# ha7ilm/csdr

Measured on AMD Instinct MI355X. Metric: complex MS/s in->out, WFM demod chain @2.4 MS/s x N streams, higher is better.
Workload: dtype f32

## Files before the change

csdr_amd/__init__.py:

```python
import ctypes as C
import os
import sys
import subprocess
import numpy as np

HERE = os.path.dirname(os.path.abspath(__file__))
LIB_PATH = os.environ.get("CSDR_AMD_LIB") or os.path.join(HERE, "libcsdr_amd.so")
ROOT = os.path.dirname(HERE)

c64 = np.complex64
f32 = np.float32

SHIFT = {"addition": 0, "math": 1, "table": 2, "unroll": 3, "addfast": 4}
WINDOWS = {"BOXCAR": 0, "BLACKMAN": 1, "HAMMING": 2}


class CsdrAmdError(RuntimeError):
    pass


def build(verbose=False):
    r = subprocess.run(["make", "-C", os.path.join(HERE, "csrc"), "-j8"], capture_output=True, text=True)
    if r.returncode != 0:
        raise CsdrAmdError("libcsdr_amd build failed:\n" + r.stdout[-4000:] + r.stderr[-4000:])
# ... 305 lines not shown
    L.csdr_amd_loopback_destroy.argtypes = [vp]; L.csdr_amd_loopback_destroy.restype = None
    L.csdr_amd_loopback_abort.argtypes = [vp]; L.csdr_amd_loopback_abort.restype = None
    L.csdr_amd_comm_create_loopback.restype = vp; L.csdr_amd_comm_create_loopback.argtypes = [vp, vp, i]
    L.csdr_amd_comm_create_null.restype = vp; L.csdr_amd_comm_create_null.argtypes = [vp, i, i]
    L.csdr_amd_comm_create_ipc.restype = vp; L.csdr_amd_comm_create_ipc.argtypes = [vp, C.c_char_p, i, i]
    L.csdr_amd_fastddc_inv_kernel_name.restype = C.c_char_p; L.csdr_amd_fastddc_inv_kernel_name.argtypes = [vp]
    L.csdr_amd_fastddc_inv_kernels.restype = C.c_char_p; L.csdr_amd_fastddc_inv_kernels.argtypes = [vp]
    L.csdr_amd_fastddc_inv_set_profiling.argtypes = [vp, i]
    L.csdr_amd_fastddc_inv_kernel_time.argtypes = [vp, C.POINTER(C.c_double), C.POINTER(C.c_long)]
    L.csdr_amd_fastddc_inv_stage_time.argtypes = [vp, i, C.POINTER(C.c_double), C.POINTER(C.c_long)]
    L.csdr_amd_wfm_create.restype = vp; L.csdr_amd_wfm_create.argtypes = [vp, i, fl, i, vp, i, i, fl, i, sz]
    L.csdr_amd_wfm_destroy.argtypes = [vp]
    L.csdr_amd_wfm_reset.argtypes = [vp]
    L.csdr_amd_wfm_process.restype = C.c_long; L.csdr_amd_wfm_process.argtypes = [vp, vp, sz, sz, vp, vp, sz]
    L.csdr_amd_wfm_kernel_name.restype = C.c_char_p; L.csdr_amd_wfm_kernel_name.argtypes = [vp]
    ll = C.c_longlong; db = C.c_double
    L.csdr_amd_wfm_ring_create.restype = vp; L.csdr_amd_wfm_ring_create.argtypes = [vp, i, fl, i, vp, i, i, fl, i, sz, i]
    L.csdr_amd_wfm_ring_destroy.argtypes = [vp]; L.csdr_amd_wfm_ring_destroy.restype = None
    L.csdr_amd_wfm_ring_reset.argtypes = [vp]
    L.csdr_amd_wfm_ring_acquire.argtypes = [vp, ll, db]
    L.csdr_amd_wfm_ring_input.restype = vp; L.csdr_amd_wfm_ring_input.argtypes = [vp, ll, C.POINTER(sz)]
    L.csdr_amd_wfm_ring_submit.restype = ll; L.csdr_amd_wfm_ring_submit.argtypes = [vp]
    L.csdr_amd_wfm_ring_wait.restype = C.c_long; L.csdr_amd_wfm_ring_wait.argtypes = [vp, ll, db]
    L.csdr_amd_wfm_ring_output.restype = vp; L.csdr_amd_wfm_ring_output.argtypes = [vp, ll, C.POINTER(sz)]
    L.csdr_amd_wfm_ring_set_rate.argtypes = [vp, fl]
    L.csdr_amd_wfm_ring_get_rate.restype = fl; L.csdr_amd_wfm_ring_get_rate.argtypes = [vp]
    L.csdr_amd_wfm_ring_set_timeouts.argtypes = [vp, db, db]
    L.csdr_amd_wfm_ring_resident.argtypes = [vp]
    L.csdr_amd_wfm_ring_stop.argtypes = [vp]
    L.csdr_amd_wfm_ring_slots.argtypes = [vp]
# ... 2610 lines not shown
```

csdr_amd/csrc/wfm.hip:

```cpp
#include "common.hpp"
#include "wfm_mfma.hpp"
#include "seeds.hpp"
#include <math.h>
#include <stdlib.h>
#include <vector>
#include <string>
#include <string.h>
using namespace csdr_amd;

namespace {

constexpr int HIST = WFM_HIST;
constexpr int TILE_A = 64;
constexpr int WARM = 48;

struct WfmParams {
    int D, L, F;
    int T;
    long long B;
    long long j_first;
    int n_audio;
};

__device__ __forceinline__ float u8_to_f(uint32_t v) { return fmaf((float)v, 0x1.010102p-7f, -1.0f); }
// ... 149 lines not shown
    bool ended;
    std::string kernel_name;
    bool profiling;
    KernelTimer timer;
    double prof_ms; long prof_launches;
    bool use_mfma;
    WfmMfmaDevice mfma;
    DevBuf<> seq_frags; DevBuf<float> seq_cum; DevBuf<float2> dtab;
    DevBuf<float2> d_ctab; size_t ctab_cap;
    float2 c_prev;
    long long tab_first; bool tab_valid;
    long tabs_built;
    bool ps; std::vector<float> rates, h_taps; DevBuf<float> d_scales;
    DevBuf<float2> d_dtab_old; DevBuf<int> d_lead_n; int *d_list; DevBuf<float> d_lead_d; std::vector<int> retuned;
    Owned<csdr_amd::SeedTables, seeds_destroy> seeds;
};

extern "C" {

static int wfm_upload_stream_tables(csdr_amd_wfm *w, int s, float rate)
{
    WfmMfmaTable t;
    wfm_mfma_build_table(w->D, w->L, w->F, rate, w->h_taps.data(), t);
    CSDR_HIP(hipMemcpy((uint8_t *)w->mfma.d_seq_frags + (size_t)s * t.seq_frags.size(), t.seq_frags.data(), t.seq_frags.size(), hipMemcpyHostToDevice));
    CSDR_HIP(hipMemcpy(w->mfma.d_seq_cum + (size_t)s * t.seq_cum.size(), t.seq_cum.data(), t.seq_cum.size() * sizeof(float), hipMemcpyHostToDevice));
    CSDR_HIP(hipMemcpy(w->mfma.d_dtab + (size_t)s * t.dtab.size(), t.dtab.data(), t.dtab.size() * sizeof(float2), hipMemcpyHostToDevice));
    CSDR_HIP(hipMemcpy(w->d_scales.get() + s, &t.seq_scale, sizeof(float), hipMemcpyHostToDevice));
    return 0;
}

// ... 115 lines not shown
    CSDR_HIP(hipMemsetAsync(w->d_last[1].get(), 0, sizeof(float) * w->n_streams, st));
    if (w->d_rot) CSDR_HIP(hipMemsetAsync(w->d_rot.get(), 0, sizeof(cf32) * (HIST + w->max_block + 64), st));
    if (w->d_hist) CSDR_HIP(hipMemsetAsync(w->d_hist.get(), 0x80, (size_t)2 * HIST * w->n_streams, st));
    for (int k = 0; k < 2; k++) if (w->d_head[k]) CSDR_HIP(hipMemsetAsync(w->d_head[k].get(), 0x80, wfm_mfma_head_bytes(w->n_streams), st));
    w->hflip = 0;
    w->B = 0; w->next_j = 0; w->last_T = 0; w->flip = 0; w->ended = false;
    w->c_prev = make_float2(1.f, 0.f); w->tab_valid = false; w->tab_first = 0;
    w->retuned.clear();
    if (w->seeds) { const int rc = seeds_reset(w->seeds.get()); if (rc) return rc; }
    return 0;
}

const char *csdr_amd_wfm_kernel_name(const csdr_amd_wfm *w) { return w->kernel_name.c_str(); }
int csdr_amd_wfm_fallback(const csdr_amd_wfm *w) { return w->use_mfma ? 0 : 1; }

int csdr_amd_wfm_seed_stats(const csdr_amd_wfm *w, long out[5])
{
    if (!w || !out) return fail_msg(-3, "wfm_seed_stats: bad arguments");
    if (!w->ps) return fail_msg(-3, "wfm_seed_stats: the object shares one rate, it has no per-stream seed tables (csdr_amd_wfm_tables_built counts its host-built table)");
    seeds_stats(w->seeds.get(), out);
    return 0;
}

long csdr_amd_wfm_tables_built(const csdr_amd_wfm *w)
{
    if (!w) return fail_msg(-3, "wfm_tables_built: bad arguments");
    if (!w->ps) return w->tabs_built;
    long st[5]; seeds_stats(w->seeds.get(), st);
    return st[0];
}
// ... 94 lines not shown
                if (n_lead > n_audio) n_lead = n_audio;
            }
            if (n_lead > 0) {
                const int nr = (int)w->retuned.size(), S = w->n_streams;
                if (!w->d_lead_n) { CSDR_HIP(dev_alloc(w->d_lead_n, sizeof(int) * 2 * S)); w->d_list = w->d_lead_n.get() + S; CSDR_HIP(dev_alloc(w->d_lead_d, sizeof(float) * (size_t)lead_max * S)); }
                int *hl = (int *)c->pinned_acquire(sizeof(int) * (size_t)(S + nr)); if (!hl) return -2;
                for (int s = 0; s < S; s++) hl[s] = 0;
                for (int k = 0; k < nr; k++) { hl[w->retuned[k]] = (int)n_lead; hl[S + k] = w->retuned[k]; }
                rc = c->pinned_upload(w->d_lead_n.get(), sizeof(int) * (size_t)(S + nr)); if (rc) return rc;
                rc = wfm_mfma_lead(st, in, in_pitch, back.head_in, w->d_taps.get(), sv.ctab, sv.pitch, w->mfma.d_dtab, w->d_dtab_old.get(), w->d_list, nr, w->d_lead_d.get(), lead_max,
                                   w->D, w->L, w->F, w->B, w->next_j, (int)n_lead);
                if (rc) return rc;
                psa.d_lead_d = w->d_lead_d.get(); psa.d_lead_n = w->d_lead_n.get();
            }
        }
        rc = wfm_mfma_launch(st, e0, e1, in, in_pitch, w->mfma, ctab_call, w->n_streams, T, w->B, w->next_j, n_audio, back, w->ps ? &psa : nullptr);
        if (rc) return rc;
        if (n_audio > 0) w->retuned.clear();
        w->hflip ^= 1;
        if (n_audio > 0) w->flip ^= 1;
    } else {
        if ((size_t)n_audio + 40 > w->demod_pitch) return fail_msg(-3, "wfm: internal audio buffer too small");
        if (n_audio > 0) {
            WfmParams p; p.D = w->D; p.L = w->L; p.F = w->F; p.T = T; p.B = w->B; p.j_first = w->next_j; p.n_audio = n_audio;
            const int span = w->D * (w->F * (TILE_A - 1) + 1) + w->L + 16;
            const size_t lds = (size_t)((span + 7) / 8 * 8 + 2 * TILE_A) * sizeof(float2) + 64;
            if (lds > 64 * 1024) { const int arc = lds_attr_once((const void *)k_wfm_front, lds); if (arc) return arc; }
            if (e0) CSDR_HIP(hipEventRecord(e0, st));
            hipLaunchKernelGGL(k_wfm_front, dim3(w->n_streams, cdiv(n_audio, TILE_A)), dim3(256), lds, st,
                               in, in_pitch, w->d_hist.get(), w->d_rot.get(), w->d_taps.get(), w->d_demod.get(), w->demod_pitch, p);
            CSDR_LAUNCH_CHECK();
// ... 18 lines not shown
```

csdr_amd/csrc/wfm_mfma.hip:

```cpp
#include "common.hpp"
#include "wfm_mfma.hpp"
#include <hip/hip_ext.h>
#include <math.h>
#include <string.h>
#include <stdlib.h>
#include <complex>
#include <vector>
using namespace csdr_amd;

namespace csdr_amd {

bool wfm_mfma_supported(int D, int L, int F)
{
    if ((D * F) & 1) return false;
    const int win_off = (18 * D) & ~15;
    const int span_bytes = 2 * (D * (3 * F + 10) + L) - win_off;
    if (span_bytes > 64 * WFM_NK) return false;
    if (D + L + 3 * D * F + 8 > WFM_HIST) return false;
    return true;
}

void wfm_mfma_build_table(int D, int L, int F, float shift_rate, const float *taps, WfmMfmaTable &t)
{
    t.D = D; t.L = L; t.F = F;
// ... 97 lines not shown
            for (int l = 0; l < 3; l++) acc[l] = __builtin_amdgcn_mfma_i32_16x16x64_i8(A[ks * 3 + l], Bf[ks], acc[l], 0, 0, 0);
        }
    }
}

struct SeqParams {
    int n_streams; long long B2; long long tile_first; int n_tiles, tiles_per_seg;
    int stride, win_off; float scale;
    long long two_T;
    float alpha; const float *last_in; float *last_out; int16_t *s16; float *af; size_t out_pitch; long long j_first; int n_audio;
    const uint8_t *head_in; uint8_t *head_out;
    long long col_bytes; int col_chunks, col_audio, n_cols;
    size_t frag_stride, tab_pitch; int tab_len;
    const float *scales;
    const float *lead_d; const int *lead_n; int lead_stride;
};

#ifndef SEQ_RB_KIB
#define SEQ_RB_KIB 9
#endif
constexpr int SEQ_RB = 1024 * SEQ_RB_KIB;
#ifndef SEQ_RING_PAD
#define SEQ_RING_PAD 32
#endif
constexpr int SEQ_RP = SEQ_RB + SEQ_RING_PAD;
constexpr int SEQ_NGR = 4 * WFM_NK;
#ifndef SEQ_TPG_N
#define SEQ_TPG_N 6
#endif
#ifndef SEQ_NLD_N
// ... 29 lines not shown
    unsigned *cnt;
    unsigned long long *t_first;
    unsigned long long *next_item;
    unsigned *exiting;
    const uint8_t *in_ring; int16_t *out_ring; size_t in_slot_bytes, out_slot_elems;
    int n_slots, desc_lines, n_wsb, T, D, L, F;
    long long idle_ticks, life_ticks;
    const float *lead_d; int lead_stride;
    const float *lead_state;
    unsigned long long *stats;
    int fence_mode;
};
__device__ __forceinline__ uint32_t sys_load(const uint32_t *p) { return __hip_atomic_load(p, __ATOMIC_RELAXED, __HIP_MEMORY_SCOPE_SYSTEM); }
__device__ __forceinline__ uint32_t res_tag(long long k) { return (uint32_t)((unsigned long long)k % 0xfffffffeull) + 1u; }

template <bool PS, bool RES = false>
__global__ __launch_bounds__(64 * SEQ_NW) void k_wfm_mfma_seq(const uint8_t *__restrict__ in, size_t in_pitch, const v4i *__restrict__ frags, const float *__restrict__ cum,
                                                               const float2 *__restrict__ dtab, const float2 *__restrict__ ctab, SeqParams p_in, ResCtl rc)
{
    static_assert(!(PS && RES), "the resident form exists for the shared-rate kernel");
    constexpr int TPG = SEQ_TPG, SPW = 16 / SEQ_NLW, NTHR = 64 * SEQ_NW;
    extern __shared__ float4 lds_raw[];
    uint8_t *lds_in = reinterpret_cast<uint8_t *>(lds_raw);
    float *lds_out = reinterpret_cast<float *>(lds_in + 16 * SEQ_RP);
    float *lcum = lds_out + 16 * SEQ_OUTP;
    float2 *ctl = reinterpret_cast<float2 *>(lcum + (SEQ_NGR + 1) * 16);
    const int tid = threadIdx.x, wv = __builtin_amdgcn_readfirstlane(tid >> 6), lane = tid & 63, col = lane & 15, q = lane >> 4;
    const bool fetches = wv >= TPG;
#ifdef WFM_PROF
    const long long t_entry = __builtin_readcyclecounter();
    long long t_first = t_entry, t_last = t_entry;
#endif
    const int fw = wv - TPG;
    float scale = p_in.scale;
    if constexpr (PS) { const int sbp = blockIdx.x; frags += (size_t)sbp * p_in.frag_stride; cum += (size_t)sbp * ((SEQ_NGR + 1) * 16); dtab += (size_t)sbp * 3072; ctab += sbp; scale = p_in.scales[sbp]; }
    for (int i = tid; i < (SEQ_NGR + 1) * 16; i += NTHR) lcum[i] = cum[i];
    v4i A[WFM_NK * 3];
#pragma unroll
    for (int s = 0; s < WFM_NK * 3; s++) A[s] = frags[s * 64 + lane];

    float c_lo[4], c_hi[4];
    {
        const float4 a = *reinterpret_cast<const float4 *>(cum + 4 * q), b = *reinterpret_cast<const float4 *>(cum + (size_t)SEQ_NGR * 16 + 4 * q);
        c_lo[0] = a.x; c_lo[1] = a.y; c_lo[2] = a.z; c_lo[3] = a.w; c_hi[0] = b.x; c_hi[1] = b.y; c_hi[2] = b.z; c_hi[3] = b.w;
    }
    const float K = 0.340447550238101026565118445432744920253753662109375f;
    SeqParams p_res;
    if constexpr (RES) p_res = p_in;
    const SeqParams &p = RES ? p_res : p_in;
    unsigned long long item = 0;
    long long res_t_launch = 0;
    uint32_t *const rctl = reinterpret_cast<uint32_t *>(ctl);
    const float2 *const lseed = ctl + 1;
    long long st_wait = 0, st_body = 0, st_done = 0, st_items = 0, st_t = 0;
    if constexpr (RES) { item = rc.next_item[blockIdx.x]; res_t_launch = wall_clock64(); st_t = res_t_launch; }
    bool pend = false; unsigned pend_c = 0; int pend_slot = 0, pend_n = 0; long long pend_k = 0;
    uint32_t pre_v[4] = {0u, 0u, 0u, 0u}; bool pre_valid = false;
    auto res_complete = [&]() {
        if constexpr (RES) {
            if (tid == 0 && pend) {
                pend = false;
                if (pend_c + 1 == (unsigned)rc.n_wsb) {
                    const unsigned long long tf = __hip_atomic_exchange(rc.t_first + pend_slot, ~0ull, __ATOMIC_RELAXED, __HIP_MEMORY_SCOPE_AGENT), td = (unsigned long long)wall_clock64();
                    __hip_atomic_store(rc.cnt + pend_slot, 0u, __ATOMIC_RELAXED, __HIP_MEMORY_SCOPE_AGENT);
                    uint32_t *dn = rc.done + (size_t)pend_slot * 16;
                    __hip_atomic_store(dn + 1, (uint32_t)pend_n, __ATOMIC_RELAXED, __HIP_MEMORY_SCOPE_SYSTEM);
                    __hip_atomic_store(dn + 2, (uint32_t)tf, __ATOMIC_RELAXED, __HIP_MEMORY_SCOPE_SYSTEM); __hip_atomic_store(dn + 3, (uint32_t)(tf >> 32), __ATOMIC_RELAXED, __HIP_MEMORY_SCOPE_SYSTEM);
                    __hip_atomic_store(dn + 4, (uint32_t)td, __ATOMIC_RELAXED, __HIP_MEMORY_SCOPE_SYSTEM); __hip_atomic_store(dn + 5, (uint32_t)(td >> 32), __ATOMIC_RELAXED, __HIP_MEMORY_SCOPE_SYSTEM);
                    asm volatile("s_waitcnt vmcnt(0)" ::: "memory");
                    __hip_atomic_store(dn, res_tag(pend_k), __ATOMIC_RELAXED, __HIP_MEMORY_SCOPE_SYSTEM);
// ... 66 lines not shown
        auto j_hi = [&](long long kk) -> long long {
            if (kk < 0) return -1;
            const long long avail_last = (kk + 1) * rc.T - 1;
            if (avail_last - (rc.L - 1) < 0) return -1;
            const long long k_max = (avail_last - (rc.L - 1)) / rc.D;
            return k_max >= 10 ? (k_max - 10) / rc.F : -1;
        };
        const long long jp = j_hi(res_k - 1), jn = j_hi(res_k);
        p_res.B2 = 2 * res_k * rc.T;
        p_res.j_first = jp + 1; p_res.n_audio = (int)(jn - jp);
        p_res.tile_first = p_res.j_first / 4; p_res.n_tiles = (int)((p_res.j_first + p_res.n_audio - 1) / 4 - p_res.tile_first + 1);
        p_res.tiles_per_seg = p_res.n_tiles;
        p_res.s16 = rc.out_ring + (size_t)res_slot * rc.out_slot_elems;
        if (tid == 0) (void)__hip_atomic_fetch_min(rc.t_first + res_slot, (unsigned long long)wall_clock64(), __ATOMIC_RELAXED, __HIP_MEMORY_SCOPE_AGENT);
    }
    const int sb = RES ? (int)(item % (unsigned)rc.n_wsb) : (int)blockIdx.x;
    const int seg_y = RES ? 0 : (int)blockIdx.y;
    const int col0 = PS ? 16 * seg_y : 0;
    if constexpr (RES) {
        in = rc.in_ring + (size_t)res_slot * rc.in_slot_bytes;
        pblock = rc.in_ring + (size_t)((res_slot + rc.n_slots - 1) % rc.n_slots) * rc.in_slot_bytes + (long long)sb * 16 * (long long)in_pitch;
    }
    const long long t0 = p.tile_first + (long long)seg_y * p.tiles_per_seg * (PS ? 16 : 1);
    long long t1 = t0 + p.tiles_per_seg; if (t1 > p.tile_first + p.n_tiles) t1 = p.tile_first + p.n_tiles;
    if (!RES && t0 >= t1) return;
    const int n_it = (int)(t1 - t0), n_grp = (n_it + TPG - 1) / TPG;
    const int n_lead = RES ? res_lead : ((PS && p.lead_n && seg_y == 0) ? p.lead_n[sb] : 0);
    const int n_warm = RES ? ((res_k > 0 && !res_retuned) ? 2 : 0) : ((PS || seg_y > 0) ? 2 : 0);
    const int last_stream = p.n_streams - 1;
    const int tstride = p.stride;
    const long long org = PS ? (long long)col0 * p.col_bytes : 0LL;
    long long wg = (t0 - (long long)n_warm * TPG) * tstride + p.win_off - p.B2 - org;
// ... 177 lines not shown
            const int srow = ei / SPS, k = ei % SPS, kr = g * SPS + k;
            if (ei >= 16 * SPS) continue;
            if (PS ? (kr < col_lo(srow) || kr >= col_hi(srow)) : (kr < seg_lo || kr >= seg_hi || s0 + srow >= p.n_streams)) continue;
            const float e = lds_out[srow * SEQ_OUTP + (g % SEQ_OUTS) * SPS + k];
            const long long idx = idx0 + kr;
            const size_t at = PS ? (size_t)sb * p.out_pitch + (size_t)srow * p.col_audio + idx : (size_t)(s0 + srow) * p.out_pitch + idx;
            p.s16[at] = (int16_t)s16_of(e);
            if (p.af) p.af[at] = e;
        }
    };
#ifdef WFM_PROF
    long long prof[8] = {0, 0, 0, 0, 0, 0, 0, 0}, t_prev = __builtin_readcyclecounter();
#endif
    if (fetches) {
        typedef unsigned wfm_u4 __attribute__((ext_vector_type(4)));
        constexpr int NST = RES ? 8 : 44;
#define WFM_ST_ALL(X) X(0) X(1) X(2) X(3) X(4) X(5) X(6) X(7) X(8) X(9) X(10) X(11) X(12) X(13) X(14) X(15) X(16) X(17) X(18) X(19) X(20) X(21) X(22) X(23) \
                      X(24) X(25) X(26) X(27) X(28) X(29) X(30) X(31) X(32) X(33) X(34) X(35) X(36) X(37) X(38) X(39) X(40) X(41) X(42) X(43)
#define X(k) wfm_u4 st##k = {0u, 0u, 0u, 0u};
        WFM_ST_ALL(X)
#undef X
        int n_st = 0, st_n0 = 0;
        const int srow = 8 * fw + (lane >> 3), pc = lane & 7;
        const int lo_r = col_lo(srow), hi_r = col_hi(srow);
        const bool row_ok = PS ? hi_r > lo_r : s0 + srow < p.n_streams;
        const size_t row_at = PS ? (size_t)sb * p.out_pitch + (size_t)srow * p.col_audio : (size_t)(s0 + srow) * p.out_pitch;
        int16_t *const orow = p.s16 + row_at;
        auto flush = [&]() __attribute__((always_inline)) {
            if constexpr (PS) {
#define X(j) if (j < NST && j < n_st && row_ok) { const int a = st_n0 + SEQ_LINE * j + 8 * pc;                                                             \
                 if (a + 8 <= hi_r) *reinterpret_cast<uint4 *>(orow + (idx0 + a)) = make_uint4(st##j[0], st##j[1], st##j[2], st##j[3]);        \
// ... 56 lines not shown
            if (gi + 1 < n_grp) { while (F < F_end && F + 1024 <= wg_n + SEQ_RB) row_step(); }
            PROF_T(3)
            if (WFM_DIAG < 4) take_line(gi - 1);
            PROF_T(4)
#ifdef WFM_PROF
            prof[6] += 1;
#endif
            wg = wg_n;
        }
#ifdef WFM_PROF
        if (lane == 0) for (int k = 0; k < 8; k++) atomicAdd(&g_wfm_prof[wv][k], (unsigned long long)prof[k]);
        t_last = __builtin_readcyclecounter();
#endif
        __syncthreads();
        if (WFM_DIAG < 4) { take_line(n_grp - 1); take_line(n_grp); flush(); }
#undef WFM_ST_ALL
    } else {
    PROF_T(7)
#ifdef WFM_PROF
    t_first = __builtin_readcyclecounter();
#endif
    for (int gi = -n_warm; gi < n_grp; gi++) {
        const int it = gi * TPG + wv;
        float *lout = lds_out + ((gi + SEQ_OUTS) % SEQ_OUTS) * SPS;
        if (it < n_it && (WFM_DIAG < 3)) {
            const long long ws = wg + (long long)wv * tstride;
            const long long n0 = (ws + p.B2) >> 1;
            const int off = (int)(n0 & 1023);
            const bool two = off + 32 * WFM_NK > 1024;
            const int bo = 2 * (1024 - off);
// ... 117 lines not shown
    }
#ifdef WFM_PROF
    if (lane == 0) for (int k = 0; k < 8; k++) atomicAdd(&g_wfm_prof[wv][k], (unsigned long long)prof[k]);
    t_last = __builtin_readcyclecounter();
#endif
    __syncthreads();
    if (!emit_vec) emit_scalar(n_grp - 1);
    }
    if (PS && seg_y + 1 == (int)gridDim.y) {
        if (iir_lane && col0 + lane == p.n_cols - 1) p.last_out[sb] = yst;
        if (tid < 32 && p.two_T >= 512 && (p.two_T & 15) == 0) {
            const uint4 v = *reinterpret_cast<const uint4 *>(in + (size_t)sb * in_pitch + (p.two_T - 512) + 16 * tid);
            *reinterpret_cast<uint4 *>(p.head_out + (size_t)sb * SEQ_HEAD + 512 + 16 * tid) = v;
        }
    } else
    if (!PS && !RES && seg_y + 1 == (int)gridDim.y) {
        if (iir_lane && s0 + lane < p.n_streams) p.last_out[s0 + lane] = yst;
        if (tid < 16 * 32 && p.two_T >= 512 && (p.two_T & 15) == 0 && s0 + tid / 32 < p.n_streams) {
            const int srow = tid / 32, piece = tid % 32;
            const uint4 v = *reinterpret_cast<const uint4 *>(sblock + (size_t)srow * in_pitch + (p.two_T - 512) + 16 * piece);
            *reinterpret_cast<uint4 *>(p.head_out + (size_t)(s0 + srow) * SEQ_HEAD + 512 + 16 * piece) = v;
        }
    }
#ifdef WFM_PROF
    if (lane == 0) {
        asm volatile("s_waitcnt vmcnt(0)" ::: "memory");
        const long long t_exit = __builtin_readcyclecounter();
        atomicAdd(&g_wfm_life[wv][0], (unsigned long long)(t_first - t_entry)); atomicAdd(&g_wfm_life[wv][1], (unsigned long long)(t_last - t_first));
        atomicAdd(&g_wfm_life[wv][2], (unsigned long long)(t_exit - t_last)); atomicAdd(&g_wfm_life[wv][3], 1ULL);
    }
#endif
    if constexpr (!RES) break;
    else {
        if (tid == 0) { const long long t = wall_clock64(); st_body += t - st_t; st_t = t; }
        if (wv == 0) {
            const unsigned long long nx = item + gridDim.x;
            const long long nk = (long long)(nx / (unsigned)rc.n_wsb);
            const uint32_t *dsc = rc.desc + (size_t)(nk % rc.n_slots) * rc.desc_lines * 16;
            const int nd = rc.desc_lines * 16;
#pragma unroll
            for (int j = 0; j < 4; j++) { const int d = lane + 64 * j; pre_v[j] = d < nd ? sys_load(dsc + d) : 0u; }
            pre_valid = true;
        }
        if (rc.fence_mode == 2) __threadfence_system();
        if (wv != 0 || !emit_vec) asm volatile("s_waitcnt vmcnt(0)" ::: "memory");
        __syncthreads();
        if (tid == 0) {
// ... 81 lines not shown
                         const float2 *d_dtab_old, const int *d_list, int n_list, float *d_lead_d, int lead_stride, float *d_warm, float *d_state, float alpha,
                         int D, int L, int F, long long B, long long j_first, int n_lead)
{
    if (n_list <= 0) return 0;
    if (j_first < RES_WARM) return fail_msg(-3, "wfm ring: a retune needs %d audio samples in front of the block", RES_WARM);
    LeadParams lp; lp.D = D; lp.L = L; lp.F = F; lp.B = B; lp.j_first = j_first; lp.n_lead = n_lead; lp.tab_pitch = 1; lp.dtab_stride = 0;
    lp.ct_stride = 0; lp.head_pitch = in_pitch; lp.head_off = two_T - 512; lp.c_first = (B >> 10) - 4; lp.ja0 = -RES_WARM; lp.warm = d_warm; lp.lead_stride = lead_stride;
    hipLaunchKernelGGL(k_wfm_lead, dim3(n_lead + RES_WARM, n_list), dim3(128), 0, st, in, in_pitch, prev, d_taps, ctab, d_dtab, d_dtab_old, d_list, d_lead_d, lp);
    CSDR_LAUNCH_CHECK();
    hipLaunchKernelGGL(k_wfm_lead_state, dim3((n_list + 63) / 64), dim3(64), 0, st, d_warm, d_state, n_list, alpha);
    CSDR_LAUNCH_CHECK();
    return 0;
}

int wfm_mfma_launch(hipStream_t st, hipEvent_t ev_begin, hipEvent_t ev_end, const uint8_t *in, size_t in_pitch, const WfmMfmaDevice &dev, const float2 *ctab,
                    int n_streams, int T, long long B, long long j_first, int n_audio, const WfmBackArgs &back, const WfmPerStream *ps)
{
    if (in_pitch * 16 + 4096 >= ((size_t)1 << 32)) return fail_msg(-3, "wfm: in_pitch %zu too large for the matrix-core front end (32-bit row offsets)", in_pitch);
    if (n_audio <= 0) {
        hipLaunchKernelGGL(k_wfm_roll_head, dim3(n_streams), dim3(256), 0, st, in, in_pitch, 2LL * T, back.head_in, back.head_out);
        CSDR_LAUNCH_CHECK();
        return 0;
    }
    SeqParams sp;
    memset((void *)&sp, 0, sizeof sp);
    ResCtl no_res; memset((void *)&no_res, 0, sizeof no_res);
    sp.n_streams = n_streams; sp.B2 = 2 * B; sp.two_T = 2LL * T;
    sp.tile_first = j_first / 4; sp.n_tiles = (int)((j_first + n_audio - 1) / 4 - sp.tile_first + 1);
    sp.stride = dev.tile_stride_bytes; sp.win_off = dev.win_off_bytes; sp.scale = dev.seq_scale;
    const int n_cu = current_device_cu_count();
    const int n_wsb = (n_streams + 15) / 16;
    int n_seg = (n_cu + n_wsb - 1) / n_wsb; if (n_seg < 1) n_seg = 1;
// ... 13 lines not shown
        int np = (n_per + 16 * n_ss - 1) / (16 * n_ss); if (np < 1) np = 1;
        sp.tiles_per_seg = np * tpp;
        sp.n_cols = (sp.n_tiles + sp.tiles_per_seg - 1) / sp.tiles_per_seg;
        n_seg = (sp.n_cols + 15) / 16;
        sp.col_bytes = (long long)sp.tiles_per_seg * sp.stride; sp.col_chunks = (int)(sp.col_bytes / 2048); sp.col_audio = 4 * sp.tiles_per_seg;
        sp.frag_stride = (size_t)WFM_NK * 3 * 64; sp.tab_pitch = ps->tab_pitch; sp.tab_len = ps->tab_len; sp.scales = ps->d_scales;
        sp.lead_d = ps->d_lead_d; sp.lead_n = ps->d_lead_n; sp.lead_stride = ps->lead_stride;
        if (sp.col_bytes * 16 + 4096 >= (1LL << 32)) return fail_msg(-3, "wfm: block too large for the per-stream kernel's 32-bit row offsets");
        const size_t ldsp = (size_t)16 * SEQ_RP + 16 * SEQ_OUTP * sizeof(float) + (SEQ_NGR + 1) * 16 * sizeof(float) + 2 * 48 * sizeof(float2);
        { const int arc = lds_attr_once((const void *)k_wfm_mfma_seq<true>, ldsp); if (arc) return arc; }
        if (ev_begin && ev_end)
            hipExtLaunchKernelGGL(k_wfm_mfma_seq<true>, dim3(n_streams, n_seg), dim3(64 * SEQ_NW), ldsp, st, ev_begin, ev_end, 0, in, in_pitch, (const v4i *)dev.d_seq_frags, dev.d_seq_cum, dev.d_dtab, ctab, sp, no_res);
        else
            hipLaunchKernelGGL(k_wfm_mfma_seq<true>, dim3(n_streams, n_seg), dim3(64 * SEQ_NW), ldsp, st, in, in_pitch, (const v4i *)dev.d_seq_frags, dev.d_seq_cum, dev.d_dtab, ctab, sp, no_res);
        CSDR_LAUNCH_CHECK();
        if (T < 256 || (T & 7)) {
            hipLaunchKernelGGL(k_wfm_roll_head, dim3(n_streams), dim3(256), 0, st, in, in_pitch, 2LL * T, back.head_in, back.head_out);
            CSDR_LAUNCH_CHECK();
        }
        return 0;
    }
    const size_t lds = (size_t)16 * SEQ_RP + 16 * SEQ_OUTP * sizeof(float) + (SEQ_NGR + 1) * 16 * sizeof(float);
    { const int arc = lds_attr_once((const void *)k_wfm_mfma_seq<false>, lds); if (arc) return arc; }
    if (ev_begin && ev_end)
        hipExtLaunchKernelGGL(k_wfm_mfma_seq<false>, dim3(n_wsb, n_seg), dim3(64 * SEQ_NW), lds, st, ev_begin, ev_end, 0, in, in_pitch, (const v4i *)dev.d_seq_frags, dev.d_seq_cum, dev.d_dtab, ctab, sp, no_res);
    else
        hipLaunchKernelGGL(k_wfm_mfma_seq<false>, dim3(n_wsb, n_seg), dim3(64 * SEQ_NW), lds, st, in, in_pitch, (const v4i *)dev.d_seq_frags, dev.d_seq_cum, dev.d_dtab, ctab, sp, no_res);
    CSDR_LAUNCH_CHECK();
    if (T < 256 || (T & 7)) {
        hipLaunchKernelGGL(k_wfm_roll_head, dim3(n_streams), dim3(256), 0, st, in, in_pitch, 2LL * T, back.head_in, back.head_out);
        CSDR_LAUNCH_CHECK();
    }
    return 0;
}

int wfm_mfma_launch_resident(hipStream_t st, hipEvent_t ev_end, const WfmMfmaDevice &dev, int n_streams, size_t in_pitch, float alpha, size_t out_pitch, const WfmResident &rv, int grid)
{
// ... 83 lines not shown
```

csdr_amd/csrc/wfm_mfma.hpp:

```cpp
#pragma once
#include "common.hpp"
#include <vector>

namespace csdr_amd {

constexpr int WFM_HIST = 256;
constexpr int WFM_NK = 8;

struct WfmMfmaTable {
    int D, L, F, tile_stride_bytes, win_off_bytes;
    std::vector<int8_t> seq_frags;
    std::vector<float> seq_cum;
    std::vector<float2> dtab;
    float seq_scale;
};

struct WfmMfmaDevice {
    int tile_stride_bytes, win_off_bytes;
    void *d_seq_frags; float *d_seq_cum; float2 *d_dtab; float seq_scale;
};

struct WfmBackArgs {
    float alpha; const float *last_in; float *last_out; int16_t *s16; float *af; size_t out_pitch; const uint8_t *head_in; uint8_t *head_out;
};
// ... 8 lines not shown
    int n_slots, desc_lines, T, D, L, F;
    long long idle_ticks, life_ticks;
    const float *lead_d, *lead_state; int lead_stride;
    unsigned long long *stats; int fence_mode;
};
constexpr int WFM_RES_WARM = 48;
int wfm_mfma_launch_resident(hipStream_t st, hipEvent_t ev_end, const WfmMfmaDevice &dev, int n_streams, size_t in_pitch, float alpha, size_t out_pitch, const WfmResident &rv, int grid);
int wfm_resident_max_grid();
int wfm_mfma_lead_shared(hipStream_t st, const uint8_t *in, size_t in_pitch, const uint8_t *prev, size_t two_T, const float *d_taps, const float2 *ctab, const float2 *d_dtab,
                         const float2 *d_dtab_old, const int *d_list, int n_list, float *d_lead_d, int lead_stride, float *d_warm, float *d_state, float alpha,
                         int D, int L, int F, long long B, long long j_first, int n_lead);

bool wfm_mfma_supported(int D, int L, int F);
void wfm_mfma_build_table(int D, int L, int F, float shift_rate, const float *taps, WfmMfmaTable &t);
size_t wfm_mfma_head_bytes(int n_streams);
int wfm_mfma_launch(hipStream_t st, hipEvent_t ev_begin, hipEvent_t ev_end, const uint8_t *in, size_t in_pitch, const WfmMfmaDevice &dev, const float2 *ctab,
                    int n_streams, int T, long long B, long long j_first, int n_audio, const WfmBackArgs &back, const WfmPerStream *ps = nullptr);
int wfm_mfma_lead(hipStream_t st, const uint8_t *in, size_t in_pitch, const uint8_t *head, const float *d_taps, const float2 *ctab, size_t tab_pitch, const float2 *d_dtab,
                  const float2 *d_dtab_old, const int *d_list, int n_list, float *d_lead_d, int lead_stride, int D, int L, int F, long long B, long long j_first, int n_lead);

}
```

include/csdr_amd.h:

```cpp
#ifndef CSDR_AMD_H
#define CSDR_AMD_H
#include <stddef.h>
#include <stdint.h>

#ifdef __cplusplus
extern "C" {
#endif

typedef struct csdr_complexf_s { float i, q; } csdr_complexf;

typedef enum { CSDR_WINDOW_BOXCAR = 0, CSDR_WINDOW_BLACKMAN = 1, CSDR_WINDOW_HAMMING = 2 } csdr_window_t;

typedef struct csdr_amd_ctx csdr_amd_ctx;

csdr_amd_ctx *csdr_amd_ctx_create(int device, void *hip_stream);
void          csdr_amd_ctx_destroy(csdr_amd_ctx *ctx);
int           csdr_amd_ctx_sync(csdr_amd_ctx *ctx);
void         *csdr_amd_ctx_stream(csdr_amd_ctx *ctx);
const char   *csdr_amd_last_error(void);
int           csdr_amd_device_count(void);
const char   *csdr_amd_device_arch(csdr_amd_ctx *ctx);

void *csdr_amd_malloc(csdr_amd_ctx *ctx, size_t bytes);
void  csdr_amd_free(csdr_amd_ctx *ctx, void *dptr);
// ... 568 lines not shown
typedef struct csdr_amd_wfm csdr_amd_wfm;
csdr_amd_wfm *csdr_amd_wfm_create(csdr_amd_ctx *ctx, int n_streams, float shift_rate, int decimation,
                                  const float *host_taps, int taps_length, int frac_rate,
                                  float tau, int audio_rate, size_t max_block_samples);
csdr_amd_wfm *csdr_amd_wfm_create_rates(csdr_amd_ctx *ctx, int n_streams, const float *shift_rates, int decimation,
                                        const float *host_taps, int taps_length, int frac_rate,
                                        float tau, int audio_rate, size_t max_block_samples);
int   csdr_amd_wfm_set_rate(csdr_amd_wfm *w, int stream, float shift_rate);
float csdr_amd_wfm_get_rate(const csdr_amd_wfm *w, int stream);
void csdr_amd_wfm_destroy(csdr_amd_wfm *w);
int  csdr_amd_wfm_reset(csdr_amd_wfm *w);
long csdr_amd_wfm_process(csdr_amd_wfm *w, const uint8_t *in, size_t in_pitch, size_t block_samples,
                          int16_t *audio_s16, float *audio_f, size_t out_pitch);
const char *csdr_amd_wfm_kernel_name(const csdr_amd_wfm *w);
int csdr_amd_wfm_fallback(const csdr_amd_wfm *w);
int  csdr_amd_wfm_seed_stats(const csdr_amd_wfm *w, long out[5]);
long csdr_amd_wfm_tables_built(const csdr_amd_wfm *w);
int csdr_amd_wfm_set_profiling(csdr_amd_wfm *w, int on);
int csdr_amd_wfm_kernel_time(csdr_amd_wfm *w, double *total_ms, long *launches);

typedef struct csdr_amd_wfm_ring csdr_amd_wfm_ring;
csdr_amd_wfm_ring *csdr_amd_wfm_ring_create(csdr_amd_ctx *ctx, int n_streams, float shift_rate, int decimation, const float *host_taps, int taps_length, int frac_rate,
                                            float tau, int audio_rate, size_t block_samples, int n_slots);
void csdr_amd_wfm_ring_destroy(csdr_amd_wfm_ring *r);
int  csdr_amd_wfm_ring_reset(csdr_amd_wfm_ring *r);
int  csdr_amd_wfm_ring_acquire(csdr_amd_wfm_ring *r, long long seq, double timeout_s);
uint8_t *csdr_amd_wfm_ring_input(csdr_amd_wfm_ring *r, long long seq, size_t *pitch_bytes);
long long csdr_amd_wfm_ring_submit(csdr_amd_wfm_ring *r);
long csdr_amd_wfm_ring_wait(csdr_amd_wfm_ring *r, long long seq, double timeout_s);
const int16_t *csdr_amd_wfm_ring_output(csdr_amd_wfm_ring *r, long long seq, size_t *pitch_samples);
// ... 114 lines not shown
```

Baseline: 2.933 million.

## Add persistent grid-stride walk launch for shared-rate WFM matrix-core kernel

Adds a WALK variant of the sequential MFMA WFM kernel. It launches one workgroup per CU by default and has each workgroup loop over (stream-block, segment) items with a grid stride. Fetch waves skip loading the A fragments and cum tables, and the fetch-side staging register count drops from 44 to 36, which frees registers and overlaps setup. The last-segment tail work (IIR state, head copy) is moved into the walk loop. This is meant to cut launch and tail overhead when there are more items than CUs, at the cost of serializing items per workgroup and extra barriers.

Result: no change. 2.926 million (-0.2%).

```diff
diff --git a/csdr_amd/__init__.py b/csdr_amd/__init__.py
--- a/csdr_amd/__init__.py
+++ b/csdr_amd/__init__.py
@@ -343,6 +343,9 @@
     L.csdr_amd_wfm_reset.argtypes = [vp]
     L.csdr_amd_wfm_process.restype = C.c_long; L.csdr_amd_wfm_process.argtypes = [vp, vp, sz, sz, vp, vp, sz]
     L.csdr_amd_wfm_kernel_name.restype = C.c_char_p; L.csdr_amd_wfm_kernel_name.argtypes = [vp]
+    if hasattr(L, "csdr_amd_wfm_set_walk"):
+        L.csdr_amd_wfm_set_walk.argtypes = [vp, i]
+        L.csdr_amd_wfm_last_launch.argtypes = [vp, C.POINTER(C.c_int), C.POINTER(C.c_int)]
     ll = C.c_longlong; db = C.c_double
     L.csdr_amd_wfm_ring_create.restype = vp; L.csdr_amd_wfm_ring_create.argtypes = [vp, i, fl, i, vp, i, i, fl, i, sz, i]
     L.csdr_amd_wfm_ring_destroy.argtypes = [vp]; L.csdr_amd_wfm_ring_destroy.restype = None
diff --git a/csdr_amd/csrc/wfm.hip b/csdr_amd/csrc/wfm.hip
--- a/csdr_amd/csrc/wfm.hip
+++ b/csdr_amd/csrc/wfm.hip
@@ -187,6 +187,8 @@
     bool ps; std::vector<float> rates, h_taps; DevBuf<float> d_scales;
     DevBuf<float2> d_dtab_old; DevBuf<int> d_lead_n; int *d_list; DevBuf<float> d_lead_d; std::vector<int> retuned;
     Owned<csdr_amd::SeedTables, seeds_destroy> seeds;
+    int walk = 0;
+    WfmLaunchInfo last_launch = {0, 0};
 };
 
 extern "C" {
@@ -332,6 +334,21 @@
 const char *csdr_amd_wfm_kernel_name(const csdr_amd_wfm *w) { return w->kernel_name.c_str(); }
 int csdr_amd_wfm_fallback(const csdr_amd_wfm *w) { return w->use_mfma ? 0 : 1; }
 
+int csdr_amd_wfm_set_walk(csdr_amd_wfm *w, int grid)
+{
+    if (!w || grid < -1) return fail_msg(-3, "wfm_set_walk: bad arguments");
+    w->walk = grid;
+    return 0;
+}
+
+int csdr_amd_wfm_last_launch(const csdr_amd_wfm *w, int *workgroups, int *items)
+{
+    if (!w) return fail_msg(-3, "wfm_last_launch: bad arguments");
+    if (workgroups) *workgroups = w->last_launch.workgroups;
+    if (items) *items = w->last_launch.items;
+    return 0;
+}
+
 int csdr_amd_wfm_seed_stats(const csdr_amd_wfm *w, long out[5])
 {
     if (!w || !out) return fail_msg(-3, "wfm_seed_stats: bad arguments");
@@ -456,7 +473,8 @@
                 psa.d_lead_d = w->d_lead_d.get(); psa.d_lead_n = w->d_lead_n.get();
             }
         }
-        rc = wfm_mfma_launch(st, e0, e1, in, in_pitch, w->mfma, ctab_call, w->n_streams, T, w->B, w->next_j, n_audio, back, w->ps ? &psa : nullptr);
+        rc = wfm_mfma_launch(st, e0, e1, in, in_pitch, w->mfma, ctab_call, w->n_streams, T, w->B, w->next_j, n_audio, back, w->ps ? &psa : nullptr,
+                             w->walk, &w->last_launch);
         if (rc) return rc;
         if (n_audio > 0) w->retuned.clear();
         w->hflip ^= 1;
diff --git a/csdr_amd/csrc/wfm_mfma.hip b/csdr_amd/csrc/wfm_mfma.hip
--- a/csdr_amd/csrc/wfm_mfma.hip
+++ b/csdr_amd/csrc/wfm_mfma.hip
@@ -135,6 +135,7 @@
     size_t frag_stride, tab_pitch; int tab_len;
     const float *scales;
     const float *lead_d; const int *lead_n; int lead_stride;
+    int walk_wsb, walk_items;
 };
 
 #ifndef SEQ_RB_KIB
@@ -194,11 +195,12 @@
 __device__ __forceinline__ uint32_t sys_load(const uint32_t *p) { return __hip_atomic_load(p, __ATOMIC_RELAXED, __HIP_MEMORY_SCOPE_SYSTEM); }
 __device__ __forceinline__ uint32_t res_tag(long long k) { return (uint32_t)((unsigned long long)k % 0xfffffffeull) + 1u; }
 
-template <bool PS, bool RES = false>
+template <bool PS, bool RES = false, bool WALK = false>
 __global__ __launch_bounds__(64 * SEQ_NW) void k_wfm_mfma_seq(const uint8_t *__restrict__ in, size_t in_pitch, const v4i *__restrict__ frags, const float *__restrict__ cum,
                                                                const float2 *__restrict__ dtab, const float2 *__restrict__ ctab, SeqParams p_in, ResCtl rc)
 {
     static_assert(!(PS && RES), "the resident form exists for the shared-rate kernel");
+    static_assert(!WALK || (!PS && !RES), "the walk belongs to the launched shared-rate kernel");
     constexpr int TPG = SEQ_TPG, SPW = 16 / SEQ_NLW, NTHR = 64 * SEQ_NW;
     extern __shared__ float4 lds_raw[];
     uint8_t *lds_in = reinterpret_cast<uint8_t *>(lds_raw);
@@ -208,21 +210,24 @@
     const int tid = threadIdx.x, wv = __builtin_amdgcn_readfirstlane(tid >> 6), lane = tid & 63, col = lane & 15, q = lane >> 4;
     const bool fetches = wv >= TPG;
 #ifdef WFM_PROF
-    const long long t_entry = __builtin_readcyclecounter();
+    long long t_entry = __builtin_readcyclecounter();
     long long t_first = t_entry, t_last = t_entry;
 #endif
     const int fw = wv - TPG;
     float scale = p_in.scale;
     if constexpr (PS) { const int sbp = blockIdx.x; frags += (size_t)sbp * p_in.frag_stride; cum += (size_t)sbp * ((SEQ_NGR + 1) * 16); dtab += (size_t)sbp * 3072; ctab += sbp; scale = p_in.scales[sbp]; }
-    for (int i = tid; i < (SEQ_NGR + 1) * 16; i += NTHR) lcum[i] = cum[i];
+    constexpr bool FETCH_FIRST = WALK;
     v4i A[WFM_NK * 3];
-#pragma unroll
-    for (int s = 0; s < WFM_NK * 3; s++) A[s] = frags[s * 64 + lane];
-
-    float c_lo[4], c_hi[4];
-    {
+    float c_lo[4] = {0.f, 0.f, 0.f, 0.f}, c_hi[4] = {0.f, 0.f, 0.f, 0.f};
+    if (!FETCH_FIRST || !fetches) {
+        for (int i = tid; i < (SEQ_NGR + 1) * 16; i += (FETCH_FIRST ? 64 * TPG : NTHR)) lcum[i] = cum[i];
+#pragma unroll
+        for (int s = 0; s < WFM_NK * 3; s++) A[s] = frags[s * 64 + lane];
         const float4 a = *reinterpret_cast<const float4 *>(cum + 4 * q), b = *reinterpret_cast<const float4 *>(cum + (size_t)SEQ_NGR * 16 + 4 * q);
         c_lo[0] = a.x; c_lo[1] = a.y; c_lo[2] = a.z; c_lo[3] = a.w; c_hi[0] = b.x; c_hi[1] = b.y; c_hi[2] = b.z; c_hi[3] = b.w;
+    } else {
+#pragma unroll
+        for (int s = 0; s < WFM_NK * 3; s++) A[s] = v4i{0, 0, 0, 0};
     }
     const float K = 0.340447550238101026565118445432744920253753662109375f;
     SeqParams p_res;
@@ -234,6 +239,7 @@
     const float2 *const lseed = ctl + 1;
     long long st_wait = 0, st_body = 0, st_done = 0, st_items = 0, st_t = 0;
     if constexpr (RES) { item = rc.next_item[blockIdx.x]; res_t_launch = wall_clock64(); st_t = res_t_launch; }
+    unsigned witem = blockIdx.x;
     bool pend = false; unsigned pend_c = 0; int pend_slot = 0, pend_n = 0; long long pend_k = 0;
     uint32_t pre_v[4] = {0u, 0u, 0u, 0u}; bool pre_valid = false;
     auto res_complete = [&]() {
@@ -330,8 +336,8 @@
         p_res.s16 = rc.out_ring + (size_t)res_slot * rc.out_slot_elems;
         if (tid == 0) (void)__hip_atomic_fetch_min(rc.t_first + res_slot, (unsigned long long)wall_clock64(), __ATOMIC_RELAXED, __HIP_MEMORY_SCOPE_AGENT);
     }
-    const int sb = RES ? (int)(item % (unsigned)rc.n_wsb) : (int)blockIdx.x;
-    const int seg_y = RES ? 0 : (int)blockIdx.y;
+    const int sb = RES ? (int)(item % (unsigned)rc.n_wsb) : (WALK ? (int)(witem % (unsigned)p.walk_wsb) : (int)blockIdx.x);
+    const int seg_y = RES ? 0 : (WALK ? (int)(witem / (unsigned)p.walk_wsb) : (int)blockIdx.y);
     const int col0 = PS ? 16 * seg_y : 0;
     if constexpr (RES) {
         in = rc.in_ring + (size_t)res_slot * rc.in_slot_bytes;
@@ -539,7 +545,7 @@
 #endif
     if (fetches) {
         typedef unsigned wfm_u4 __attribute__((ext_vector_type(4)));
-        constexpr int NST = RES ? 8 : 44;
+        constexpr int NST = RES ? 8 : (WALK ? 36 : 44);
 #define WFM_ST_ALL(X) X(0) X(1) X(2) X(3) X(4) X(5) X(6) X(7) X(8) X(9) X(10) X(11) X(12) X(13) X(14) X(15) X(16) X(17) X(18) X(19) X(20) X(21) X(22) X(23) \
                       X(24) X(25) X(26) X(27) X(28) X(29) X(30) X(31) X(32) X(33) X(34) X(35) X(36) X(37) X(38) X(39) X(40) X(41) X(42) X(43)
 #define X(k) wfm_u4 st##k = {0u, 0u, 0u, 0u};
@@ -626,6 +632,12 @@
 #endif
         __syncthreads();
         if (WFM_DIAG < 4) { take_line(n_grp - 1); take_line(n_grp); flush(); }
+        if constexpr (WALK) {
+#pragma unroll
+            for (int s = 0; s < WFM_NK * 3; s++) asm volatile("" : "=v"(A[s]));
+#pragma unroll
+            for (int r = 0; r < 4; r++) asm volatile("" : "=v"(c_lo[r]), "=v"(c_hi[r]));
+        }
 #undef WFM_ST_ALL
     } else {
     PROF_T(7)
@@ -773,7 +785,7 @@
             *reinterpret_cast<uint4 *>(p.head_out + (size_t)sb * SEQ_HEAD + 512 + 16 * tid) = v;
         }
     } else
-    if (!PS && !RES && seg_y + 1 == (int)gridDim.y) {
+    if (!PS && !RES && !WALK && seg_y + 1 == (int)gridDim.y) {
         if (iir_lane && s0 + lane < p.n_streams) p.last_out[s0 + lane] = yst;
         if (tid < 16 * 32 && p.two_T >= 512 && (p.two_T & 15) == 0 && s0 + tid / 32 < p.n_streams) {
             const int srow = tid / 32, piece = tid % 32;
@@ -789,7 +801,25 @@
         atomicAdd(&g_wfm_life[wv][2], (unsigned long long)(t_exit - t_last)); atomicAdd(&g_wfm_life[wv][3], 1ULL);
     }
 #endif
-    if constexpr (!RES) break;
+    if constexpr (WALK) {
+        const bool more = witem + gridDim.x < (unsigned)p.walk_items;
+        if (more) __syncthreads();
+        if (!fetches && witem + (unsigned)p.walk_wsb >= (unsigned)p.walk_items) {
+            if (iir_lane && s0 + lane < p.n_streams) p.last_out[s0 + lane] = yst;
+            if (p.two_T >= 512 && (p.two_T & 15) == 0)
+                for (int e = tid; e < 16 * 32; e += 64 * TPG) {
+                    const int srow = e / 32, piece = e % 32;
+                    if (s0 + srow >= p.n_streams) continue;
+                    const uint4 v = *reinterpret_cast<const uint4 *>(sblock + (size_t)srow * in_pitch + (p.two_T - 512) + 16 * piece);
+                    *reinterpret_cast<uint4 *>(p.head_out + (size_t)(s0 + srow) * SEQ_HEAD + 512 + 16 * piece) = v;
+                }
+        }
+        if (!more) break;
+        witem += gridDim.x;
+#ifdef WFM_PROF
+        t_entry = __builtin_readcyclecounter();
+#endif
+    } else if constexpr (!RES) break;
     else {
         if (tid == 0) { const long long t = wall_clock64(); st_body += t - st_t; st_t = t; }
         if (wv == 0) {
@@ -901,8 +931,9 @@
 }
 
 int wfm_mfma_launch(hipStream_t st, hipEvent_t ev_begin, hipEvent_t ev_end, const uint8_t *in, size_t in_pitch, const WfmMfmaDevice &dev, const float2 *ctab,
-                    int n_streams, int T, long long B, long long j_first, int n_audio, const WfmBackArgs &back, const WfmPerStream *ps)
-{
+                    int n_streams, int T, long long B, long long j_first, int n_audio, const WfmBackArgs &back, const WfmPerStream *ps, int walk, WfmLaunchInfo *info)
+{
+    if (info) { info->workgroups = 0; info->items = 0; }
     if (in_pitch * 16 + 4096 >= ((size_t)1 << 32)) return fail_msg(-3, "wfm: in_pitch %zu too large for the matrix-core front end (32-bit row offsets)", in_pitch);
     if (n_audio <= 0) {
         hipLaunchKernelGGL(k_wfm_roll_head, dim3(n_streams), dim3(256), 0, st, in, in_pitch, 2LL * T, back.head_in, back.head_out);
@@ -946,6 +977,7 @@
         else
             hipLaunchKernelGGL(k_wfm_mfma_seq<true>, dim3(n_streams, n_seg), dim3(64 * SEQ_NW), ldsp, st, in, in_pitch, (const v4i *)dev.d_seq_frags, dev.d_seq_cum, dev.d_dtab, ctab, sp, no_res);
         CSDR_LAUNCH_CHECK();
+        if (info) { info->workgroups = n_streams * n_seg; info->items = n_streams * n_seg; }
         if (T < 256 || (T & 7)) {
             hipLaunchKernelGGL(k_wfm_roll_head, dim3(n_streams), dim3(256), 0, st, in, in_pitch, 2LL * T, back.head_in, back.head_out);
             CSDR_LAUNCH_CHECK();
@@ -953,6 +985,23 @@
         return 0;
     }
     const size_t lds = (size_t)16 * SEQ_RP + 16 * SEQ_OUTP * sizeof(float) + (SEQ_NGR + 1) * 16 * sizeof(float);
+    const int n_items = n_wsb * n_seg, walk_grid = walk > 0 ? walk : n_cu;
+    if (walk >= 0 && n_items > walk_grid) {
+        sp.walk_wsb = n_wsb; sp.walk_items = n_items;
+        { const int arc = lds_attr_once((const void *)k_wfm_mfma_seq<false, false, true>, lds); if (arc) return arc; }
+        if (ev_begin && ev_end)
+            hipExtLaunchKernelGGL((k_wfm_mfma_seq<false, false, true>), dim3(walk_grid), dim3(64 * SEQ_NW), lds, st, ev_begin, ev_end, 0, in, in_pitch, (const v4i *)dev.d_seq_frags, dev.d_seq_cum, dev.d_dtab, ctab, sp, no_res);
+        else
+            hipLaunchKernelGGL((k_wfm_mfma_seq<false, false, true>), dim3(walk_grid), dim3(64 * SEQ_NW), lds, st, in, in_pitch, (const v4i *)dev.d_seq_frags, dev.d_seq_cum, dev.d_dtab, ctab, sp, no_res);
+        CSDR_LAUNCH_CHECK();
+        if (info) { info->workgroups = walk_grid; info->items = n_items; }
+        if (T < 256 || (T & 7)) {
+            hipLaunchKernelGGL(k_wfm_roll_head, dim3(n_streams), dim3(256), 0, st, in, in_pitch, 2LL * T, back.head_in, back.head_out);
+            CSDR_LAUNCH_CHECK();
+        }
+        return 0;
+    }
+    if (info) { info->workgroups = n_items; info->items = n_items; }
     { const int arc = lds_attr_once((const void *)k_wfm_mfma_seq<false>, lds); if (arc) return arc; }
     if (ev_begin && ev_end)
         hipExtLaunchKernelGGL(k_wfm_mfma_seq<false>, dim3(n_wsb, n_seg), dim3(64 * SEQ_NW), lds, st, ev_begin, ev_end, 0, in, in_pitch, (const v4i *)dev.d_seq_frags, dev.d_seq_cum, dev.d_dtab, ctab, sp, no_res);
diff --git a/csdr_amd/csrc/wfm_mfma.hpp b/csdr_amd/csrc/wfm_mfma.hpp
--- a/csdr_amd/csrc/wfm_mfma.hpp
+++ b/csdr_amd/csrc/wfm_mfma.hpp
@@ -46,8 +46,10 @@
 bool wfm_mfma_supported(int D, int L, int F);
 void wfm_mfma_build_table(int D, int L, int F, float shift_rate, const float *taps, WfmMfmaTable &t);
 size_t wfm_mfma_head_bytes(int n_streams);
+struct WfmLaunchInfo { int workgroups, items; };
 int wfm_mfma_launch(hipStream_t st, hipEvent_t ev_begin, hipEvent_t ev_end, const uint8_t *in, size_t in_pitch, const WfmMfmaDevice &dev, const float2 *ctab,
-                    int n_streams, int T, long long B, long long j_first, int n_audio, const WfmBackArgs &back, const WfmPerStream *ps = nullptr);
+                    int n_streams, int T, long long B, long long j_first, int n_audio, const WfmBackArgs &back, const WfmPerStream *ps = nullptr, int walk = 0,
+                    WfmLaunchInfo *info = nullptr);
 int wfm_mfma_lead(hipStream_t st, const uint8_t *in, size_t in_pitch, const uint8_t *head, const float *d_taps, const float2 *ctab, size_t tab_pitch, const float2 *d_dtab,
                   const float2 *d_dtab_old, const int *d_list, int n_list, float *d_lead_d, int lead_stride, int D, int L, int F, long long B, long long j_first, int n_lead);
 
diff --git a/include/csdr_amd.h b/include/csdr_amd.h
--- a/include/csdr_amd.h
+++ b/include/csdr_amd.h
@@ -606,6 +606,8 @@
                           int16_t *audio_s16, float *audio_f, size_t out_pitch);
 const char *csdr_amd_wfm_kernel_name(const csdr_amd_wfm *w);
 int csdr_amd_wfm_fallback(const csdr_amd_wfm *w);
+int csdr_amd_wfm_set_walk(csdr_amd_wfm *w, int grid);
+int csdr_amd_wfm_last_launch(const csdr_amd_wfm *w, int *workgroups, int *items);
 int  csdr_amd_wfm_seed_stats(const csdr_amd_wfm *w, long out[5]);
 long csdr_amd_wfm_tables_built(const csdr_amd_wfm *w);
 int csdr_amd_wfm_set_profiling(csdr_amd_wfm *w, int on);
```
